# cfdeinza/reinforcement-learning-rendezvous

Hardware: AMD Instinct MI355X
Metric: env steps/sec (higher is better)
Workload: dtype f64

## Files before the change

### reinforcement_learning_rendezvous_amd/csrc/rdv_fused.h

```cpp
#pragma once
#include "rdv_kernels.h"

namespace rdv {

template <typename ST, bool kDiag, bool kGeneral = false, bool kRaw = false>
__global__ __launch_bounds__(kBlock) void step_kernel(void* ws_hot, const float* actions_hot, const DevParams* __restrict__ Pp, int64_t n_hot,
                                                       uint64_t* stats_hot, float* obs_hot, float* reward_hot, const StepArgs A_rest) {
  const StepArgs A = hot_args(A_rest, ws_hot, actions_hot, n_hot, stats_hot, obs_hot, reward_hot);
  using V = typename Vec4<ST>::type;
  __shared__ __attribute__((aligned(16))) float lds[kBlock * RDV_OBS_DIM];
  const DevParams& P = *Pp;
  const int lane = threadIdx.x & (kWave - 1);
  const int wave_in_block = threadIdx.x >> 6;
  const int64_t lblock = A.xcd_per ? (int64_t)(blockIdx.x & 7) * A.xcd_per + (blockIdx.x >> 3) : (int64_t)blockIdx.x;
  const int64_t i = lblock * kBlock + threadIdx.x;
  const int64_t wave_base = i - lane;
  const int64_t n = A.n;
  const bool active = i < n;
  const int64_t rows = (n - wave_base) < kWave ? (n - wave_base) : kWave;
  float* wl = lds + wave_in_block * (kWave * RDV_OBS_DIM);
  V* ws = reinterpret_cast<V*>(A.ws);

  Env e;
  if (active) load_env<ST>(ws, A.cs, i, e);
  uint64_t* slot = A.stats + (uint64_t)(wave_base / kWave) * kStatWords;
  const uint64_t slot_pre = rows > 0 ? stats_preload(slot, lane) : 0ull;
  float a[RDV_ACT_DIM];
  load_actions(A.actions, wave_base, lane, active, a);

  StepResult r;
  const RowSink my_row{wl + lane * RDV_OBS_DIM};
  const bool stepped = advance<ST, kDiag, kGeneral, kRaw>(A, P, i, active, e, a, r, my_row);
  const bool fin = stepped && r.done;
  stats_update(slot, slot_pre, lane, stepped, fin, r.reason, e.flags, e.k, e.ep_ret, e.sum_dv, e.sum_dw);
  store_step_outputs<true>(A, i, active, fin, r, e, my_row.row);
  bool did_reset = false;
  if (fin) {
    if (A.on_done == RDV_ON_DONE_RESET) {
      const double* row = nullptr;
      if (A.tape_depth > 0) row = A.tape + ((int64_t)(e.episode % (uint32_t)A.tape_depth) * n + i) * RDV_STATE_DIM;
      reset_env<ST>(P, e, A.seed, A.env_id_offset + (uint64_t)i, row);
// ... 15 lines not shown
```

### reinforcement_learning_rendezvous_amd/csrc/rdv_general.hip

```cpp
#include "rdv_fused.h"
#include "rdv_slots.h"
#include "rdv_general.h"

namespace rdv {

constexpr int kGenEnvs = 256;
constexpr int kGenBlock = 512;
template <typename ST>
__global__ __launch_bounds__(kGenBlock) void step_kernel_general(void* ws_hot, const float* actions_hot, const DevParams* __restrict__ Pp, int64_t n_hot,
                                                                 uint64_t* stats_hot, float* obs_hot, float* reward_hot, const StepArgs A_rest) {
  const StepArgs A = hot_args(A_rest, ws_hot, actions_hot, n_hot, stats_hot, obs_hot, reward_hot);
  using V = typename Vec4<ST>::type;
  __shared__ __attribute__((aligned(16))) float stage[kGenEnvs * RDV_OBS_DIM];
  __shared__ double handoff[7 * kGenEnvs];
  const DevParams& P = *Pp;
  const int lane = threadIdx.x & (kWave - 1);
  const int wv = threadIdx.x >> 6;
  const bool env_role = wv < kGenEnvs / kWave;
  const int slot = threadIdx.x & (kGenEnvs - 1);
  const int64_t i = (int64_t)blockIdx.x * kGenEnvs + slot;
  const int64_t wave_base = i - lane;
  const int64_t n = A.n;
  const bool active = i < n;
  const int64_t rows = (n - wave_base) < kWave ? (n - wave_base) : kWave;
  V* ws = reinterpret_cast<V*>(A.ws);

  if (env_role) {
    float* wl = stage + wv * (kWave * RDV_OBS_DIM);
    Env e;
    if (active) load_env<ST>(ws, A.cs, i, e);
    uint64_t* slot_stats = A.stats + (uint64_t)(wave_base / kWave) * kStatWords;
    const uint64_t slot_pre = rows > 0 ? stats_preload(slot_stats, lane) : 0ull;
    float a[RDV_ACT_DIM];
    load_actions(A.actions, wave_base, lane, active, a);
    const bool stepping = active && !(e.flags & FLAG_HALTED);
    Derived d;
    StepCtx c;
    StepResult r;
    r.done = 0; r.reason = 0; r.reward = 0.0f; r.reward64 = 0.0;
    if (stepping) step_env_chaser<ST, true, false>(P, e, a, d, c);
    __syncthreads();
    const RowSink my_row{wl + lane * RDV_OBS_DIM};
    if (stepping) {
#pragma unroll
// ... 14 lines not shown
    if (fin) {
      if (A.on_done == RDV_ON_DONE_RESET) {
        reset_env<ST>(P, e, A.seed, A.env_id_offset + (uint64_t)i, tape_row_of(A.tape, A.tape_depth, n, i, e.episode));
        observation_to(P, e, my_row);
      } else if (A.on_done == RDV_ON_DONE_HALT) {
        e.flags |= FLAG_HALTED;
      }
    }
    wave_lds_fence();
    if (A.stream_rows) store_obs_rows<true>(A.obs, wave_base, rows, lane, wl);
    else store_obs_rows<false>(A.obs, wave_base, rows, lane, wl);
    if (stepping) store_env<ST>(ws, A.cs, i, e, true);
  } else {
    double qt[4], wt[3];
    bool stepping = false;
    if (active) {
      const V c4 = ws[4 * A.cs + i], c5 = ws[5 * A.cs + i], c6 = ws[6 * A.cs + i];
      qt[0] = c4.x; qt[1] = c4.y; qt[2] = c4.z; qt[3] = c4.w;
      wt[0] = c6.x; wt[1] = c6.y; wt[2] = c6.z;
      stepping = !(s2u(c5.z) & FLAG_HALTED);
    }
    if (stepping) {
      step_target<true, false>(P, qt, wt);
#pragma unroll
      for (int k = 0; k < 4; ++k) handoff[k * kGenEnvs + slot] = qt[k];
#pragma unroll
      for (int k = 0; k < 3; ++k) handoff[(4 + k) * kGenEnvs + slot] = wt[k];
    }
    __syncthreads();
  }
}

const char* launch_step_general(bool f32, bool diag, bool partner_waves, int64_t n, dim3 fused_grid, hipStream_t s, const DevParams* dev_params, const StepArgs& A) {
#define RDV_LAUNCH_G(GRID, BLOCK, ...) do { hipLaunchKernelGGL((__VA_ARGS__), GRID, BLOCK, 0, s, A.ws, A.actions, dev_params, A.n, A.stats, A.obs, A.reward, A); \
                                             return #__VA_ARGS__; } while (0)
  if (partner_waves && !diag) {
    const dim3 grid((unsigned)((n + kGenEnvs - 1) / kGenEnvs));
    if (f32) RDV_LAUNCH_G(grid, dim3(kGenBlock), step_kernel_general<float>); else RDV_LAUNCH_G(grid, dim3(kGenBlock), step_kernel_general<double>);
  } else {
    const dim3 block(kBlock);
    if (f32) { if (diag) RDV_LAUNCH_G(fused_grid, block, step_kernel<float, true, true>); else RDV_LAUNCH_G(fused_grid, block, step_kernel<float, false, true>); }
    else { if (diag) RDV_LAUNCH_G(fused_grid, block, step_kernel<double, true, true>); else RDV_LAUNCH_G(fused_grid, block, step_kernel<double, false, true>); }
  }
#undef RDV_LAUNCH_G
}

}
```

### reinforcement_learning_rendezvous_amd/csrc/rdv_hip.hip

```cpp
#include "rdv_device.h"
#include "rdv_policy.h"

#include <hip/hip_runtime.h>

#include <cmath>
#include <cstdarg>
#include <cstdio>
#include <cstdlib>
#include <cstring>
#include <new>
#include <vector>

#include "../../include/rdv.h"

#include "rdv_kernels.h"
#include "rdv_fused.h"
#include "rdv_slots.h"
#include "rdv_step.h"
#include "rdv_cold.h"
#include "rdv_rollout.h"
#include "rdv_step_many.h"
#include "rdv_tiles.h"
#include "rdv_general.h"

// ... 658 lines not shown
  StepArgs A;
  base_args(h, A);
  with_storage(h->storage, [&](auto st) { hipLaunchKernelGGL(reset_kernel<decltype(st)>, grid_for(h->n), dim3(kBlock), 0, s, h->dev_params, A, mask, obs_out, fresh); });
  RDV_HIP(hipGetLastError());
  if (fresh) h->prepared_ok = true;
  h->fresh = false;
  return RDV_OK;
}

int rdv_step(rdv_handle h, const float* actions, const RdvStepOut* out, void* stream) {
  RDV_CHECK_HANDLE(h);
  if (!actions || !out || !out->obs || !out->reward || !out->done)
    return fail(RDV_ERR_INVALID_ARGUMENT, "rdv_step: actions, obs, reward and done are required");
  if (h->fresh) return fail(RDV_ERR_INVALID_ARGUMENT, "rdv_step: call rdv_reset first (state is undefined until reset(), as in the reference)");
  RDV_CHECK_FAULT(h);
  if (misaligned(actions, 8) || misaligned(out->obs, 16))
    return fail(RDV_ERR_INVALID_ARGUMENT, "rdv_step: actions must be 8-byte aligned (any row of a [K,N,6] tape is) and obs 16-byte aligned");
  if (out->diag && misaligned(out->diag, 8)) return fail(RDV_ERR_INVALID_ARGUMENT, "rdv_step: diag must be 8-byte aligned");
  DeviceGuard guard(h->device);
  StepArgs A;
  base_args(h, A);
  A.actions = actions;
  A.obs = out->obs; A.reward = out->reward; A.done = out->done; A.terminal_obs = out->terminal_obs;
  A.episode_return = out->episode_return; A.episode_length = out->episode_length; A.done_reason = out->done_reason;
  A.diag = out->diag; A.eval = out->eval;
  if (A.eval && misaligned(A.eval, 8)) return fail(RDV_ERR_INVALID_ARGUMENT, "rdv_step: eval must be 8-byte aligned");
#ifdef RDV_STAMPS
  A.stamps = h->stamps;
#endif
  hipStream_t s = static_cast<hipStream_t>(stream);
  const bool raw = h->raw_state && !h->general;
  h->raw_state = false;
  const bool split = !A.diag && !A.eval && !h->general && !raw && (h->variant == RDV_VARIANT_SPLIT || (h->variant == RDV_VARIANT_AUTO && h->n <= kSplitAutoMaxEnvs));
#define RDV_LAUNCH(GRID, BLOCK, ...) do { hipLaunchKernelGGL((__VA_ARGS__), GRID, BLOCK, 0, s, A.ws, A.actions, h->dev_params, A.n, A.stats, A.obs, A.reward, A); \
                                           h->last_kernel = #__VA_ARGS__; } while (0)
#define RDV_LAUNCH_X(GRID, BLOCK, ...) RDV_LAUNCH(GRID, BLOCK, __VA_ARGS__)
#define RDV_LAUNCH_BY(GRID, BLOCK, FLAG, K) do {                                                                                   \
    if (f32) { if (FLAG) RDV_LAUNCH_X(GRID, BLOCK, K(float, true)); else RDV_LAUNCH_X(GRID, BLOCK, K(float, false)); }             \
    else { if (FLAG) RDV_LAUNCH_X(GRID, BLOCK, K(double, true)); else RDV_LAUNCH_X(GRID, BLOCK, K(double, false)); } } while (0)
#define RDV_K_SPLIT(ST, B) step_kernel_split<ST, B>
#define RDV_K_PARTS(ST, B) step_kernel_parts<ST, B>
#define RDV_K_FUSED(ST, B) step_kernel<ST, B>
#define RDV_K_RAW(ST, B) step_kernel<ST, B, false, true>
  const bool f32 = h->storage == RDV_STORAGE_F32, dg = A.diag != nullptr || A.eval != nullptr;
  if (split) {
    const dim3 grid((unsigned)((h->n + kSplitEnvs - 1) / kSplitEnvs));
    const dim3 block(kSplitBlock);
    const bool all = h->on_done != RDV_ON_DONE_HALT;
    RDV_LAUNCH_BY(grid, block, all, RDV_K_SPLIT);
  } else {
    dim3 grid = grid_for(h->n), block(kBlock);
    { static const int forced = [] { const char* x = getenv("RDV_STREAM_ROWS"); return x ? atoi(x) : -1; }();
      A.stream_rows = forced >= 0 ? (forced ? 1 : 0) : 1; }
    { static const int forced = [] { const char* x = getenv("RDV_STAGGER"); return x ? atoi(x) : -1; }();
      A.stagger = forced >= 0 ? forced : stagger_by_size(h->n); }
    if (h->xcd_order == 1 || (h->xcd_order < 0 && xcd_order_by_size(h->n))) {
      A.xcd_per = (int32_t)((grid.x + 7) / 8);
      grid = dim3((unsigned)A.xcd_per * 8u);
    }
    if (h->general) {
      h->last_kernel = launch_step_general(f32, dg, h->dev.body_general[1] != 0 && h->split_general != 0, h->n, grid, s, h->dev_params, A);
    } else if (raw) {
      RDV_LAUNCH_BY(grid, block, dg, RDV_K_RAW);
    } else if (!dg && h->variant != RDV_VARIANT_FUSED_INLANE) {
      const bool tiles = h->variant == RDV_VARIANT_FUSED_TILES && h->on_done != RDV_ON_DONE_HALT && h->tape_depth == 0;
      if (tiles) {
        unsigned g = h->tiles_grid ? (unsigned)h->tiles_grid : (unsigned)(h->n_cus * kTilesPerCU + 7) / 8u * 8u;
        const unsigned need = A.xcd_per ? (unsigned)A.xcd_per * 8u : grid.x;
        if (g > need) g = need;
        grid = dim3(g);
        h->last_kernel = launch_step_tiles(f32, grid, s, h->dev_params, A);
      } else {
        const bool all = h->on_done != RDV_ON_DONE_HALT;
        RDV_LAUNCH_BY(grid, block, all, RDV_K_PARTS);
      }
    } else {
      RDV_LAUNCH_BY(grid, block, dg, RDV_K_FUSED);
    }
  }
#undef RDV_K_RAW
#undef RDV_K_FUSED
#undef RDV_K_PARTS
#undef RDV_K_SPLIT
#undef RDV_LAUNCH_BY
#undef RDV_LAUNCH_X
#undef RDV_LAUNCH
  RDV_HIP(hipGetLastError());
  if (h->on_done == RDV_ON_DONE_RESET) h->prepared_ok = false;
// ... 200 lines not shown
```

### reinforcement_learning_rendezvous_amd/csrc/rdv_kernels.h

```cpp
#pragma once

#include "rdv_device.h"

#include <hip/hip_runtime.h>
#include <stdint.h>

#include "../../include/rdv.h"

namespace rdv {

#ifndef RDV_PARTS_WAVES
#define RDV_PARTS_WAVES 3
#endif
constexpr int kBlock = 256;
constexpr int kWave = 64;
constexpr int kChunks = 7;
constexpr int kStatWords = 16;
constexpr int64_t kXcdOrderMaxEnvs = 3145728;
static inline bool xcd_order_by_size(int64_t n) { return n <= kXcdOrderMaxEnvs && n % 65536 == 0; }
constexpr int kTilesPerCU = 3;
static inline int stagger_by_size(int64_t n) { return (n < 229376 || n >= 1310720) ? 0 : n < 393216 ? 6 : 8; }
constexpr int64_t kSplitAutoMaxEnvs = 65536;
enum { ST_STEPS = 0, ST_EPISODES, ST_SUCCESS, ST_COLLIDED, ST_REASON0, ST_REASON1, ST_REASON2, ST_REASON3,
       ST_SUM_LEN, ST_SUM_RET, ST_SUM_DV, ST_SUM_DW };

template <typename ST> struct Vec4;
template <> struct Vec4<float> { using type = float4; };
template <> struct Vec4<double> { using type = double4; };

__device__ __forceinline__ float u2s(uint32_t u, float) { return __uint_as_float(u); }
__device__ __forceinline__ double u2s(uint32_t u, double) { return __longlong_as_double((long long)u); }
__device__ __forceinline__ uint32_t s2u(float s) { return __float_as_uint(s); }
__device__ __forceinline__ uint32_t s2u(double s) { return (uint32_t)__double_as_longlong(s); }

template <typename ST>
__device__ __forceinline__ void unpack_env(const typename Vec4<ST>::type* c, Env& e) {
  e.rc[0] = c[0].x; e.rc[1] = c[0].y; e.rc[2] = c[0].z; e.vc[0] = c[0].w;
  e.vc[1] = c[1].x; e.vc[2] = c[1].y; e.wc[0] = c[1].z; e.wc[1] = c[1].w;
// ... 68 lines not shown
#define RDV_STAMP_FLUSH(wave_id)
#endif

struct StepArgs {
  void* ws;
  uint64_t* stats;
  const float* actions;
  float* obs;
  float* reward;
  uint8_t* done;
  float* terminal_obs;
  float* episode_return;
  int32_t* episode_length;
  uint8_t* done_reason;
  double* diag;
  double* eval;
  const double* tape;
  int64_t n;
  int64_t cs;
  uint64_t seed;
  uint64_t env_id_offset;
  int32_t tape_depth;
  int32_t on_done;
  void* prep;
  uint32_t* prep_tag;
  int32_t xcd_per;
  int32_t stream_rows;
  int32_t stagger;
#ifdef RDV_STAMPS
  unsigned long long* stamps;
#endif
};

__device__ __forceinline__ StepArgs hot_args(const StepArgs& rest, void* ws, const float* actions, int64_t n, uint64_t* stats, float* obs,
                                             float* reward) {
  StepArgs A = rest;
  A.ws = ws; A.actions = actions; A.n = n; A.stats = stats; A.obs = obs; A.reward = reward;
  return A;
}
__device__ __forceinline__ StepArgs wave_outputs(const StepArgs& A, int64_t wave_base) {
  StepArgs Aw = A;
  Aw.reward = A.reward + wave_base; Aw.done = A.done + wave_base;
  Aw.done_reason = A.done_reason ? A.done_reason + wave_base : nullptr;
  Aw.terminal_obs = A.terminal_obs ? A.terminal_obs + wave_base * RDV_OBS_DIM : nullptr;
  Aw.episode_return = A.episode_return ? A.episode_return + wave_base : nullptr;
  Aw.episode_length = A.episode_length ? A.episode_length + wave_base : nullptr;
  return Aw;
}
__device__ __forceinline__ void wave_lds_fence() {
  __builtin_amdgcn_fence(__ATOMIC_ACQ_REL, "wavefront");
  __builtin_amdgcn_wave_barrier();
}

__device__ __forceinline__ void load_actions(const float* __restrict__ actions, int64_t wave_base, int lane, bool active, float* a) {
  const float* row = actions + (wave_base + lane) * RDV_ACT_DIM;
#pragma unroll
  for (int k = 0; k < 3; ++k) {
    float2 v = make_float2(0.0f, 0.0f);
    if (active) v = *reinterpret_cast<const float2*>(row + 2 * k);
    a[2 * k] = v.x; a[2 * k + 1] = v.y;
  }
}

template <typename ST>
struct TileInputs {
  typename Vec4<ST>::type c[kChunks];
  float2 a[3];
  uint64_t slot_pre;
};
template <typename ST>
__device__ __forceinline__ void tile_fetch(const StepArgs& A, int64_t wave_base, int lane, TileInputs<ST>& in) {
// ... 94 lines not shown
      iv = lane == ST_REASON0 ? (uint32_t)__popcll(m_r1) : iv;
      iv = lane == ST_REASON1 ? (uint32_t)__popcll(m_r2) : iv;
      iv = lane == ST_REASON2 ? (uint32_t)__popcll(m_r3) : iv;
      iv = lane == ST_REASON3 ? (uint32_t)__popcll(m_r4) : iv;
      iv = lane == ST_SUM_LEN ? (uint32_t)s_len : iv;
      double dv = s_ret;
      dv = lane == ST_SUM_DV ? s_dv : dv;
      dv = lane == ST_SUM_DW ? s_dw : dv;
      const uint64_t as_int = pre + iv;
      const uint64_t as_real = (uint64_t)__double_as_longlong(__longlong_as_double((long long)pre) + dv);
      slot[lane] = lane <= ST_SUM_LEN ? as_int : as_real;
    }
  } else if (lane == 0) {
    slot[ST_STEPS] = pre + __popcll(m_step);
  }
}

template <typename ST, class Sink, class Pre = NoHook>
__device__ __forceinline__ void advance_all(const DevParams& P, Env& e, const float* a, StepResult& r, Sink&& sink, typename Vec4<ST>::type* packed,
                                            Pre&& pre = Pre()) {
  r.done = 0; r.reason = 0; r.reward = 0.0f; r.reward64 = 0.0;
  Derived d;
  step_env<ST, true, false, false>(P, e, a, r, d, sink, NoHook(), pre);
  if (packed) pack_env<ST>(e, packed);
}

typedef float pin_f4 __attribute__((ext_vector_type(4)));
typedef float pin_f2 __attribute__((ext_vector_type(2)));
struct PinnedInputs {
  pin_f4 c[kChunks];
  pin_f4 a4;
  pin_f2 a2;
  pin_f2 sp;
};
__device__ __forceinline__ void pinned_fetch(const StepArgs& A, int64_t wave_base, int lane, PinnedInputs& in) {
  const int64_t wb = wave_base < A.n ? wave_base : ((A.n - 1) & ~(int64_t)(kWave - 1));
  const int64_t rows = A.n - wb;
  const int l = lane < rows ? lane : 0;
  const pin_f4* wsw = reinterpret_cast<const pin_f4*>(A.ws) + wb + l;
#pragma unroll
  for (int c = 0; c < kChunks; ++c) asm volatile("global_load_dwordx4 %0, %1, off" : "=v"(in.c[c]) : "v"(wsw + c * A.cs));
  const float* row = A.actions + (wb + l) * RDV_ACT_DIM;
  asm volatile("global_load_dwordx4 %0, %2, off\n\tglobal_load_dwordx2 %1, %2, off offset:16" : "=&v"(in.a4), "=&v"(in.a2) : "v"(row));
  const uint64_t* sp = A.stats + (uint64_t)(wb / kWave) * kStatWords + (lane & (kStatWords - 1));
  asm volatile("global_load_dwordx2 %0, %1, off" : "=v"(in.sp) : "v"(sp));
}
__device__ __forceinline__ void pinned_wait_state(PinnedInputs& in) {
  asm volatile("s_waitcnt vmcnt(3)" : "+v"(in.c[0]), "+v"(in.c[1]), "+v"(in.c[2]), "+v"(in.c[3]));
  asm volatile("" : "+v"(in.c[4]), "+v"(in.c[5]), "+v"(in.c[6]));
}
__device__ __forceinline__ void pinned_wait_rest(PinnedInputs& in, double& after) { asm volatile("s_waitcnt vmcnt(0)" : "+v"(in.a4), "+v"(in.a2), "+v"(in.sp), "+v"(after)); }
__device__ __forceinline__ void pinned_unpack(const PinnedInputs& in, Env& e) {
  float4 c[kChunks];
#pragma unroll
  for (int j = 0; j < kChunks; ++j) c[j] = make_float4(in.c[j].x, in.c[j].y, in.c[j].z, in.c[j].w);
  unpack_env<float>(c, e);
}

__device__ __forceinline__ void pinned_state(const StepArgs& A, int64_t wave_base, int lane, PinnedInputs& pin, Env& e) {
  pinned_fetch(A, wave_base, lane, pin);
  pinned_wait_state(pin);
  pinned_unpack(pin, e);
}
__device__ __forceinline__ void pinned_rest(PinnedInputs& pin, double& after, float* a, uint64_t& slot_pre) {
  pinned_wait_rest(pin, after);
  a[0] = pin.a4.x; a[1] = pin.a4.y; a[2] = pin.a4.z; a[3] = pin.a4.w; a[4] = pin.a2.x; a[5] = pin.a2.y;
  slot_pre = ((uint64_t)__float_as_uint(pin.sp.y) << 32) | __float_as_uint(pin.sp.x);
}

template <typename ST>
__device__ __forceinline__ void halt_if_done(const StepArgs& A, bool fin, Env& e, typename Vec4<ST>::type* packed) {
  if (fin && A.on_done == RDV_ON_DONE_HALT) { e.flags |= FLAG_HALTED; if (packed) packed[5].z = u2s(e.flags, ST(0)); }
}

template <bool kTerminalObs>
__device__ __forceinline__ void store_step_outputs(const StepArgs& A, int64_t i, bool active, bool fin, const StepResult& r,
                                                   const Env& e, const float* row) {
  if (active) {
    A.reward[i] = r.reward;
    A.done[i] = (uint8_t)r.done;
    if (A.done_reason)
      A.done_reason[i] = (uint8_t)(r.reason | ((fin && (e.flags & FLAG_COLLIDED)) ? 16 : 0) |
                                   ((fin && (e.flags >> SUCCESS_SHIFT) != 0u) ? 32 : 0));
  }
  if (fin) {
    if (kTerminalObs && A.terminal_obs) {
      float* t = A.terminal_obs + i * RDV_OBS_DIM;
#pragma unroll
      for (int j = 0; j < RDV_OBS_DIM; ++j) t[j] = row[j];
    }
    if (A.episode_return) A.episode_return[i] = (float)e.ep_ret;
    if (A.episode_length) A.episode_length[i] = e.k;
  }
}

// ... 35 lines not shown
```

### reinforcement_learning_rendezvous_amd/csrc/rdv_step.h

```cpp
#pragma once
#include "rdv_kernels.h"
#include "rdv_slots.h"

namespace rdv {

template <typename ST>
__global__ __launch_bounds__(kBlock) void prepare_kernel(const DevParams* __restrict__ Pp, const StepArgs A) {
  using V = typename Vec4<ST>::type;
  const int64_t i = (int64_t)blockIdx.x * kBlock + threadIdx.x;
  if (i >= A.n) return;
  const V c5 = reinterpret_cast<const V*>(A.ws)[5 * A.cs + i];
  refill_whole<ST>(A, *Pp, i, s2u(c5.w));
}

template <typename ST, bool kAll>
__global__ __launch_bounds__(kBlock) __attribute__((amdgpu_waves_per_eu(sizeof(ST) == 4 ? RDV_PARTS_WAVES : 3))) void step_kernel_parts(void* ws_hot, const float* actions_hot, const DevParams* __restrict__ Pp, int64_t n_hot,
                                                             uint64_t* stats_hot, float* obs_hot, float* reward_hot, const StepArgs A_rest) {
  const StepArgs A = hot_args(A_rest, ws_hot, actions_hot, n_hot, stats_hot, obs_hot, reward_hot);
  using V = typename Vec4<ST>::type;
  __shared__ __attribute__((aligned(16))) float lds[kBlock * RDV_OBS_DIM];
  __shared__ uint32_t job_kind[kBlock];
  __shared__ uint32_t job_counter[kBlock];
  __shared__ uint16_t lists[kGroupWaves * kBlock];
  static_assert(kBlock == kGroupEnvs, "refill_pass_lds is written for 256-env workgroups");
  const DevParams& P = *Pp;
  const int lane = threadIdx.x & (kWave - 1);
  const int wave_in_block = __builtin_amdgcn_readfirstlane((int)(threadIdx.x >> 6));
  const int64_t lblock = A.xcd_per ? (int64_t)(blockIdx.x & 7) * A.xcd_per + (blockIdx.x >> 3) : (int64_t)blockIdx.x;
  const int64_t block_base = lblock * kBlock;
  const int64_t wave_base = block_base + wave_in_block * kWave;
  const int64_t n = A.n;
  const int64_t rows = (n - wave_base) < kWave ? (n - wave_base) : kWave;
  const bool active = lane < rows;
  float* wl = lds + wave_in_block * (kWave * RDV_OBS_DIM);
  V* ws = reinterpret_cast<V*>(A.ws);
  const bool resets = A.on_done == RDV_ON_DONE_RESET;
  RDV_STAMP_DECL
  RDV_STAMP(0);
  if (A.stagger && blockIdx.x < 1024u) {
    const int slot = (int)(blockIdx.x >> 8);
    for (int k = 0; k < slot * A.stagger; ++k) __builtin_amdgcn_s_sleep(8);
  }

  {
    V* wsw = ws + wave_base;
    const StepArgs Aw = wave_outputs(A, wave_base);
    Env e;
    uint64_t* slot = A.stats + (uint64_t)(wave_base / kWave) * kStatWords;
    uint64_t slot_pre;
    float a[RDV_ACT_DIM];
    constexpr bool kPinned = kAll && sizeof(ST) == 4;
    PinnedInputs pin;
    if constexpr (kPinned) {
      pinned_state(A, wave_base, lane, pin, e);
    } else if constexpr (kAll) {
      TileInputs<ST> in;
      tile_fetch<ST>(A, wave_base, lane, in);
      unpack_env<ST>(in.c, e);
      slot_pre = in.slot_pre;
#pragma unroll
      for (int k = 0; k < 3; ++k) { a[2 * k] = in.a[k].x; a[2 * k + 1] = in.a[k].y; }
    } else {
      if (active) load_env<ST>(wsw, A.cs, lane, e);
      slot_pre = rows > 0 ? stats_preload(slot, lane) : 0ull;
      load_actions(A.actions + wave_base * RDV_ACT_DIM, 0, lane, active, a);
    }
    RDV_STAMP_STATE(e);
    RDV_STAMP(1);
    StepResult r;
    const RowSink my_row{wl + lane * RDV_OBS_DIM};
    constexpr bool kPack = sizeof(ST) == 4;
    V packed[kChunks];
    bool stepped;
    auto actions_ready = [&](double& after) { if constexpr (kPinned) pinned_rest(pin, after, a, slot_pre); };
    if constexpr (kAll) { advance_all<ST>(P, e, a, r, my_row, kPack ? packed : nullptr, actions_ready); stepped = active; }
    else stepped = advance<ST, false, false, false>(A, P, wave_base + lane, active, e, a, r, my_row, NoHook(), kPack ? packed : nullptr);
    RDV_STAMP(2);
    const bool fin = stepped && r.done;
    stats_update(slot, slot_pre, lane, stepped, fin, r.reason, e.flags, e.k, e.ep_ret, e.sum_dv, e.sum_dw);
    store_step_outputs<true>(Aw, lane, active, fin, r, e, my_row.row);
    const bool to_reset = fin && resets;
    halt_if_done<ST>(A, fin, e, kPack ? packed : nullptr);
    if (resets) {
      job_kind[threadIdx.x] = to_reset ? JOB_REFILL : JOB_NONE;
      job_counter[threadIdx.x] = e.episode;
    }
    if (stepped && !to_reset) { if (kPack) store_chunks<ST>(wsw, A.cs, lane, packed, false); else store_env<ST>(wsw, A.cs, lane, e, false); }
  }
  RDV_STAMP(3);
  if (resets) {
    __syncthreads();
    RDV_STAMP(4);
    LiveStore<ST> L;
    L.ws = ws; L.rows = lds; L.cs = A.cs; L.base = block_base;
    refill_pass_lds<ST>(wave_in_block, lane, P, L, job_kind, job_counter, lists + wave_in_block * kBlock, block_base, n, A.seed,
                        A.env_id_offset, A.tape, A.tape_depth);
    RDV_STAMP(5);
    __syncthreads();
  } else {
    wave_lds_fence();
  }
  RDV_STAMP(6);
  if (A.stream_rows) store_obs_rows<true>(A.obs, wave_base, rows, lane, wl);
  else store_obs_rows<false>(A.obs, wave_base, rows, lane, wl);
  RDV_STAMP(7);
  RDV_STAMP_FLUSH((uint64_t)blockIdx.x * (kBlock / kWave) + wave_in_block)
}

constexpr int kSplitEnvs = 256;
constexpr int kSplitBlock = 512;

template <typename ST, bool kAll>
__global__ __launch_bounds__(kSplitBlock) void step_kernel_split(void* ws_hot, const float* actions_hot, const DevParams* __restrict__ Pp, int64_t n_hot,
                                                       uint64_t* stats_hot, float* obs_hot, float* reward_hot, const StepArgs A_rest) {
  const StepArgs A = hot_args(A_rest, ws_hot, actions_hot, n_hot, stats_hot, obs_hot, reward_hot);
  using V = typename Vec4<ST>::type;
  __shared__ __attribute__((aligned(16))) float stage[kSplitEnvs * RDV_OBS_DIM];
  __shared__ unsigned long long fin_mask[kSplitEnvs / kWave];
  const DevParams& P = *Pp;
  const int lane = threadIdx.x & (kWave - 1);
  const int wv = threadIdx.x >> 6;
  const bool step_role = wv < kSplitEnvs / kWave;
  const int slot_in_block = threadIdx.x & (kSplitEnvs - 1);
  const int64_t i = (int64_t)blockIdx.x * kSplitEnvs + slot_in_block;
  const int64_t wave_base = i - lane;
  const int64_t n = A.n;
  const bool active = i < n;
  const int64_t rows = (n - wave_base) < kWave ? (n - wave_base) : kWave;
  V* ws = reinterpret_cast<V*>(A.ws);
  const bool resets = A.on_done == RDV_ON_DONE_RESET;
  RDV_STAMP_DECL
  RDV_STAMP(0);

  if (step_role) {
    __builtin_amdgcn_s_setprio(2);
    float* wl = stage + wv * (kWave * RDV_OBS_DIM);
    Env e;
    StepResult r;
    uint64_t* slot = A.stats + (uint64_t)(wave_base / kWave) * kStatWords;
    uint64_t slot_pre;
    float a[RDV_ACT_DIM];
    constexpr bool kPinned = kAll && sizeof(ST) == 4;
    PinnedInputs pin;
    if constexpr (kPinned) {
      pinned_state(A, wave_base, lane, pin, e);
    } else if constexpr (kAll) {
      TileInputs<ST> in;
      tile_fetch<ST>(A, wave_base, lane, in);
      unpack_env<ST>(in.c, e);
      slot_pre = in.slot_pre;
#pragma unroll
      for (int k = 0; k < 3; ++k) { a[2 * k] = in.a[k].x; a[2 * k + 1] = in.a[k].y; }
    } else {
      if (active) load_env<ST>(ws, A.cs, i, e);
      slot_pre = stats_preload(slot, lane);
      load_actions(A.actions, wave_base, lane, active, a);
    }
    RDV_STAMP_STATE(e);
    RDV_STAMP(1);
    float obs_r[RDV_OBS_DIM];
    float* my_row = wl + lane * RDV_OBS_DIM;
    constexpr bool kPack = sizeof(ST) == 4;
    V packed[kChunks];
    auto row_sink = [&](int j, float v) { obs_r[j] = v; my_row[j] = v; };
    bool stepped;
    auto actions_ready = [&](double& after) { if constexpr (kPinned) pinned_rest(pin, after, a, slot_pre); };
    if constexpr (kAll) { advance_all<ST>(P, e, a, r, row_sink, kPack ? packed : nullptr, actions_ready); stepped = active; }
    else stepped = advance<ST, false>(A, P, i, active, e, a, r, row_sink, NoHook(), kPack ? packed : nullptr);
    RDV_STAMP(2);
    const bool fin = stepped && r.done;
    const bool to_reset = fin && resets;
    const unsigned long long m_reset = __ballot(to_reset);
    if (lane == 0) fin_mask[wv] = m_reset;
    halt_if_done<ST>(A, fin, e, kPack ? packed : nullptr);
    if (stepped && !to_reset) { if (kPack) store_chunks<ST, true>(ws, A.cs, i, packed, false); else store_env<ST>(ws, A.cs, i, e, false); }
    RDV_STAMP(3);
    __syncthreads();
    RDV_STAMP(4);
    stats_update(slot, slot_pre, lane, stepped, fin, r.reason, e.flags, e.k, e.ep_ret, e.sum_dv, e.sum_dw);
    store_step_outputs<true>(A, i, active, fin, r, e, obs_r);
    if (m_reset == 0ull) store_obs_rows<true>(A.obs, wave_base, rows, lane, wl);
    RDV_STAMP(5);
    RDV_STAMP(6);
  } else {
    Env ne;
    if (resets && active) {
      const V c5 = ws[5 * A.cs + i];
      ne.episode = s2u(c5.w);
      RDV_STAMP(1);
      const double* row = nullptr;
      if (A.tape_depth > 0) row = A.tape + ((int64_t)(ne.episode % (uint32_t)A.tape_depth) * n + i) * RDV_STATE_DIM;
      reset_state<ST, false>(P, ne, A.seed, A.env_id_offset + (uint64_t)i, row);
      reset_aux<ST>(P, ne);
      RDV_STAMP(2);
    }
    RDV_STAMP(3);
    __syncthreads();
    RDV_STAMP(4);
    const unsigned long long m_reset = fin_mask[wv - kSplitEnvs / kWave];
    if (m_reset != 0ull) {
      float* wl = stage + (wv - kSplitEnvs / kWave) * (kWave * RDV_OBS_DIM);
      if (active && ((m_reset >> lane) & 1ull)) {
        float robs[RDV_OBS_DIM];
        canon_rest<ST>(ne);
        observation(P, ne, robs);
        store_env<ST, true>(ws, A.cs, i, ne, true);
#pragma unroll
        for (int j = 0; j < RDV_OBS_DIM; ++j) wl[lane * RDV_OBS_DIM + j] = robs[j];
      }
      wave_lds_fence();
      RDV_STAMP(5);
      store_obs_rows<true>(A.obs, wave_base, rows, lane, wl);
    }
    RDV_STAMP(6);
  }
  RDV_STAMP(7);
  RDV_STAMP_FLUSH((uint64_t)blockIdx.x * 8 + wv)
}

}
```

### reinforcement_learning_rendezvous_amd/csrc/rdv_tiles.hip

```cpp
#include "rdv_kernels.h"
#include "rdv_slots.h"
#include "rdv_tiles.h"

namespace rdv {

template <typename ST>
__device__ __forceinline__ void tile_touch(TileInputs<ST>& in) {
#pragma unroll
  for (int c = 0; c < kChunks; ++c) asm volatile("" : "+v"(in.c[c].x), "+v"(in.c[c].y), "+v"(in.c[c].z), "+v"(in.c[c].w));
#pragma unroll
  for (int k = 0; k < 3; ++k) asm volatile("" : "+v"(in.a[k].x), "+v"(in.a[k].y));
  asm volatile("" : "+v"(in.slot_pre));
}

#ifndef RDV_TILES_WAVES
#define RDV_TILES_WAVES 3
#endif
template <typename ST>
__global__ __launch_bounds__(kBlock) __attribute__((amdgpu_waves_per_eu(sizeof(ST) == 4 ? RDV_TILES_WAVES : 2))) void step_kernel_tiles(void* ws_hot, const float* actions_hot, const DevParams* __restrict__ Pp, int64_t n_hot,
                                                             uint64_t* stats_hot, float* obs_hot, float* reward_hot, const StepArgs A_rest) {
  const StepArgs A = hot_args(A_rest, ws_hot, actions_hot, n_hot, stats_hot, obs_hot, reward_hot);
  using V = typename Vec4<ST>::type;
  __shared__ __attribute__((aligned(16))) float lds[kBlock * RDV_OBS_DIM];
  __shared__ uint32_t job_kind[kBlock];
  __shared__ uint32_t job_counter[kBlock];
  __shared__ uint16_t lists[kGroupWaves * kBlock];
  const int lane0 = threadIdx.x & (kWave - 1);
  const int wave_in_block = __builtin_amdgcn_readfirstlane((int)(threadIdx.x >> 6));
  const int64_t n = A.n;
  const int64_t n_tiles = (n + kBlock - 1) / kBlock;
  const int64_t stride = A.xcd_per ? (int64_t)(gridDim.x >> 3) : (int64_t)gridDim.x;
  const int64_t first = A.xcd_per ? (int64_t)(blockIdx.x >> 3) : (int64_t)blockIdx.x;
  const int64_t limit = A.xcd_per ? (int64_t)A.xcd_per : n_tiles;
  const int64_t origin = A.xcd_per ? (int64_t)(blockIdx.x & 7) * A.xcd_per : 0;
  float* wl = lds + wave_in_block * (kWave * RDV_OBS_DIM);
  V* ws = reinterpret_cast<V*>(A.ws);
  const bool resets = A.on_done == RDV_ON_DONE_RESET;

#ifdef RDV_STAMPS
  unsigned long long ph_[12] = {0, 0, 0, 0, 0, 0, 0, 0, 0, 0, 0, 0}, t_prev_ = 0;
  ph_[8] = __builtin_amdgcn_s_memrealtime();
#define TILE_PHASE(k) do { __builtin_amdgcn_sched_barrier(0); const unsigned long long now_ = __builtin_readcyclecounter(); ph_[k] += now_ - t_prev_; t_prev_ = now_; __builtin_amdgcn_sched_barrier(0); } while (0)
  t_prev_ = __builtin_readcyclecounter();
#else
#define TILE_PHASE(k)
#endif
  int64_t lt = first;
  bool have = lt < limit && origin + lt < n_tiles;
  TileInputs<ST> in;
  if (have) tile_fetch<ST>(A, (origin + lt) * kBlock + wave_in_block * kWave, lane0, in);
#pragma clang loop unroll(disable)
  while (have) {
    int lane = lane0;
    asm volatile("" : "+v"(lane));
// ... 50 lines not shown
      if (stepped && !to_reset) store_env<ST>(wsw, A.cs, lane, e, false);
    }
    TILE_PHASE(3);
    if (resets) {
      __syncthreads();
      TILE_PHASE(4);
      LiveStore<ST> L;
      L.ws = ws; L.rows = lds; L.cs = A.cs; L.base = block_base;
      refill_pass_lds<ST>(wave_in_block, lane, P, L, job_kind, job_counter, lists + wave_in_block * kBlock, block_base, n, A.seed,
                          A.env_id_offset, nullptr, 0);
      TILE_PHASE(5);
      __syncthreads();
      TILE_PHASE(6);
    } else {
      wave_lds_fence();
    }
    tile_touch<ST>(in);
    TILE_PHASE(11);
    if (A.stream_rows) store_obs_rows<true>(A.obs, wave_base, rows, lane, wl);
    else store_obs_rows<false>(A.obs, wave_base, rows, lane, wl);
    wave_lds_fence();
    TILE_PHASE(7);
  }
#ifdef RDV_STAMPS
  if (A.stamps && lane0 == 0) {
    ph_[9] = __builtin_amdgcn_s_memrealtime();
    unsigned long long* row = A.stamps + ((uint64_t)blockIdx.x * (kBlock / kWave) + wave_in_block) * 12;
    for (int k = 0; k < 12; ++k) row[k] = ph_[k];
  }
#endif
}

const char* launch_step_tiles(bool f32, dim3 grid, hipStream_t s, const DevParams* dev_params, const StepArgs& A) {
  if (f32) hipLaunchKernelGGL(step_kernel_tiles<float>, grid, dim3(kBlock), 0, s, A.ws, A.actions, dev_params, A.n, A.stats, A.obs, A.reward, A);
  else hipLaunchKernelGGL(step_kernel_tiles<double>, grid, dim3(kBlock), 0, s, A.ws, A.actions, dev_params, A.n, A.stats, A.obs, A.reward, A);
  return f32 ? "step_kernel_tiles<float>" : "step_kernel_tiles<double>";
}

}
```

Baseline: 10.31 billion.

## Pack hot kernel args and defer loading rest of StepArgs from kernarg segment

Changes the kernel signature so the hot prefix carries cs and a packed mode word (tape depth, on_done, stagger, xcd ordering) in place of obs/reward pointers. The remaining StepArgs fields are read from the kernarg segment later via manual scalar loads, after the state loads have been issued, and the kernarg cache lines are warmed with scalar loads. The reset role in the split kernel now uses an asm load of the episode word. The aim is to shorten the kernel prologue's scalar-load latency before state fetches begin, at the cost of fragile kernarg offset assumptions.

```diff
diff --git a/reinforcement_learning_rendezvous_amd/csrc/rdv_fused.h b/reinforcement_learning_rendezvous_amd/csrc/rdv_fused.h
--- a/reinforcement_learning_rendezvous_amd/csrc/rdv_fused.h
+++ b/reinforcement_learning_rendezvous_amd/csrc/rdv_fused.h
@@ -4,9 +4,8 @@
 namespace rdv {
 
 template <typename ST, bool kDiag, bool kGeneral = false, bool kRaw = false>
-__global__ __launch_bounds__(kBlock) void step_kernel(void* ws_hot, const float* actions_hot, const DevParams* __restrict__ Pp, int64_t n_hot,
-                                                       uint64_t* stats_hot, float* obs_hot, float* reward_hot, const StepArgs A_rest) {
-  const StepArgs A = hot_args(A_rest, ws_hot, actions_hot, n_hot, stats_hot, obs_hot, reward_hot);
+__global__ __launch_bounds__(kBlock) void step_kernel(RDV_HOT_PARAMS) {
+  const StepArgs A = hot_args(A_rest, RDV_HOT_HEAD);
   using V = typename Vec4<ST>::type;
   __shared__ __attribute__((aligned(16))) float lds[kBlock * RDV_OBS_DIM];
   const DevParams& P = *Pp;
diff --git a/reinforcement_learning_rendezvous_amd/csrc/rdv_general.hip b/reinforcement_learning_rendezvous_amd/csrc/rdv_general.hip
--- a/reinforcement_learning_rendezvous_amd/csrc/rdv_general.hip
+++ b/reinforcement_learning_rendezvous_amd/csrc/rdv_general.hip
@@ -7,9 +7,8 @@
 constexpr int kGenEnvs = 256;
 constexpr int kGenBlock = 512;
 template <typename ST>
-__global__ __launch_bounds__(kGenBlock) void step_kernel_general(void* ws_hot, const float* actions_hot, const DevParams* __restrict__ Pp, int64_t n_hot,
-                                                                 uint64_t* stats_hot, float* obs_hot, float* reward_hot, const StepArgs A_rest) {
-  const StepArgs A = hot_args(A_rest, ws_hot, actions_hot, n_hot, stats_hot, obs_hot, reward_hot);
+__global__ __launch_bounds__(kGenBlock) void step_kernel_general(RDV_HOT_PARAMS) {
+  const StepArgs A = hot_args(A_rest, RDV_HOT_HEAD);
   using V = typename Vec4<ST>::type;
   __shared__ __attribute__((aligned(16))) float stage[kGenEnvs * RDV_OBS_DIM];
   __shared__ double handoff[7 * kGenEnvs];
@@ -90,7 +89,7 @@
 }
 
 const char* launch_step_general(bool f32, bool diag, bool partner_waves, int64_t n, dim3 fused_grid, hipStream_t s, const DevParams* dev_params, const StepArgs& A) {
-#define RDV_LAUNCH_G(GRID, BLOCK, ...) do { hipLaunchKernelGGL((__VA_ARGS__), GRID, BLOCK, 0, s, A.ws, A.actions, dev_params, A.n, A.stats, A.obs, A.reward, A); \
+#define RDV_LAUNCH_G(GRID, BLOCK, ...) do { hipLaunchKernelGGL((__VA_ARGS__), GRID, BLOCK, 0, s, RDV_HOT_LAUNCH_ARGS(A, dev_params)); \
                                              return #__VA_ARGS__; } while (0)
   if (partner_waves && !diag) {
     const dim3 grid((unsigned)((n + kGenEnvs - 1) / kGenEnvs));
diff --git a/reinforcement_learning_rendezvous_amd/csrc/rdv_hip.hip b/reinforcement_learning_rendezvous_amd/csrc/rdv_hip.hip
--- a/reinforcement_learning_rendezvous_amd/csrc/rdv_hip.hip
+++ b/reinforcement_learning_rendezvous_amd/csrc/rdv_hip.hip
@@ -714,7 +714,7 @@
   const bool raw = h->raw_state && !h->general;
   h->raw_state = false;
   const bool split = !A.diag && !A.eval && !h->general && !raw && (h->variant == RDV_VARIANT_SPLIT || (h->variant == RDV_VARIANT_AUTO && h->n <= kSplitAutoMaxEnvs));
-#define RDV_LAUNCH(GRID, BLOCK, ...) do { hipLaunchKernelGGL((__VA_ARGS__), GRID, BLOCK, 0, s, A.ws, A.actions, h->dev_params, A.n, A.stats, A.obs, A.reward, A); \
+#define RDV_LAUNCH(GRID, BLOCK, ...) do { hipLaunchKernelGGL((__VA_ARGS__), GRID, BLOCK, 0, s, RDV_HOT_LAUNCH_ARGS(A, h->dev_params)); \
                                            h->last_kernel = #__VA_ARGS__; } while (0)
 #define RDV_LAUNCH_X(GRID, BLOCK, ...) RDV_LAUNCH(GRID, BLOCK, __VA_ARGS__)
 #define RDV_LAUNCH_BY(GRID, BLOCK, FLAG, K) do {                                                                                   \
@@ -735,7 +735,7 @@
     { static const int forced = [] { const char* x = getenv("RDV_STREAM_ROWS"); return x ? atoi(x) : -1; }();
       A.stream_rows = forced >= 0 ? (forced ? 1 : 0) : 1; }
     { static const int forced = [] { const char* x = getenv("RDV_STAGGER"); return x ? atoi(x) : -1; }();
-      A.stagger = forced >= 0 ? forced : stagger_by_size(h->n); }
+      A.stagger = forced >= 0 ? (forced < kModeStaggerMax ? forced : kModeStaggerMax) : stagger_by_size(h->n); }
     if (h->xcd_order == 1 || (h->xcd_order < 0 && xcd_order_by_size(h->n))) {
       A.xcd_per = (int32_t)((grid.x + 7) / 8);
       grid = dim3((unsigned)A.xcd_per * 8u);
diff --git a/reinforcement_learning_rendezvous_amd/csrc/rdv_kernels.h b/reinforcement_learning_rendezvous_amd/csrc/rdv_kernels.h
--- a/reinforcement_learning_rendezvous_amd/csrc/rdv_kernels.h
+++ b/reinforcement_learning_rendezvous_amd/csrc/rdv_kernels.h
@@ -3,7 +3,9 @@
 #include "rdv_device.h"
 
 #include <hip/hip_runtime.h>
+#include <stddef.h>
 #include <stdint.h>
+#include <utility>
 
 #include "../../include/rdv.h"
 
@@ -138,11 +140,103 @@
 #endif
 };
 
-__device__ __forceinline__ StepArgs hot_args(const StepArgs& rest, void* ws, const float* actions, int64_t n, uint64_t* stats, float* obs,
-                                             float* reward) {
+#ifndef RDV_HEAD_PRELOAD
+#define RDV_HEAD_PRELOAD 1
+#endif
+#ifndef RDV_HEAD_WARM
+#define RDV_HEAD_WARM 0
+#endif
+constexpr int kModeOnDoneShift = 32, kModeStaggerShift = 34, kModeXcdShift = 42;
+constexpr int kModeStaggerMax = 255;
+inline __host__ __device__ uint64_t hot_mode(const StepArgs& A) {
+  return (uint64_t)(uint32_t)A.tape_depth | (uint64_t)((uint32_t)A.on_done & 3u) << kModeOnDoneShift |
+         (uint64_t)((uint32_t)A.stagger & (uint32_t)kModeStaggerMax) << kModeStaggerShift | (uint64_t)(uint32_t)A.xcd_per << kModeXcdShift;
+}
+#if RDV_HEAD_PRELOAD
+#define RDV_HOT_PARAMS void *ws_hot, const float *actions_hot, const DevParams *__restrict__ Pp, int64_t n_hot, uint64_t *stats_hot, int64_t cs_hot, uint64_t mode_hot, const StepArgs A_rest
+#define RDV_HOT_LAUNCH_ARGS(A, P) (A).ws, (A).actions, (P), (A).n, (A).stats, (A).cs, ::rdv::hot_mode(A), (A)
+#define RDV_HOT_HEAD hot_head(ws_hot, actions_hot, n_hot, stats_hot, cs_hot, mode_hot)
+constexpr int kRestOffset = 7 * 8;
+static_assert(alignof(StepArgs) == 8, "kRestOffset: A_rest follows the hot parameters without padding");
+__device__ __forceinline__ StepArgs hot_head(void* ws, const float* actions, int64_t n, uint64_t* stats, int64_t cs, uint64_t mode) {
+  StepArgs H = {};
+  H.ws = ws; H.actions = actions; H.n = n; H.stats = stats; H.cs = cs;
+  H.tape_depth = (int32_t)(uint32_t)mode; H.on_done = (int32_t)((mode >> kModeOnDoneShift) & 3u);
+  H.stagger = (int32_t)((mode >> kModeStaggerShift) & (uint64_t)kModeStaggerMax); H.xcd_per = (int32_t)(mode >> kModeXcdShift);
+  return H;
+}
+__device__ __forceinline__ StepArgs hot_merge(StepArgs A, const StepArgs& H) {
+  A.ws = H.ws; A.actions = H.actions; A.n = H.n; A.stats = H.stats; A.cs = H.cs;
+  A.tape_depth = H.tape_depth; A.on_done = H.on_done; A.stagger = H.stagger; A.xcd_per = H.xcd_per;
+  return A;
+}
+__device__ __forceinline__ StepArgs hot_args(const StepArgs& rest, const StepArgs& H) { return hot_merge(rest, H); }
+__device__ __forceinline__ StepArgs hot_rest(const StepArgs& rest, const StepArgs& H) {
+  typedef __attribute__((address_space(4))) const uint64_t* kernarg_ptr;
+  static_assert(sizeof(StepArgs) % 8 == 0 && kRestOffset % 8 == 0, "hot_rest copies 8-byte words");
+  kernarg_ptr k = (kernarg_ptr)__builtin_amdgcn_kernarg_segment_ptr();
+  asm volatile("" : "+s"(k));
+  uint64_t w[sizeof(StepArgs) / 8];
+#pragma unroll
+  for (size_t j = 0; j < sizeof(StepArgs) / 8; ++j) w[j] = k[kRestOffset / 8 + j];
+  StepArgs A;
+  __builtin_memcpy(&A, w, sizeof(StepArgs));
+#define RDV_REST_GLOBAL(f) A.f = (decltype(A.f))(void*)(__attribute__((address_space(1))) void*)w[offsetof(StepArgs, f) / 8]
+  RDV_REST_GLOBAL(obs); RDV_REST_GLOBAL(reward); RDV_REST_GLOBAL(done); RDV_REST_GLOBAL(terminal_obs); RDV_REST_GLOBAL(episode_return);
+  RDV_REST_GLOBAL(episode_length); RDV_REST_GLOBAL(done_reason); RDV_REST_GLOBAL(diag); RDV_REST_GLOBAL(eval); RDV_REST_GLOBAL(tape);
+  RDV_REST_GLOBAL(prep); RDV_REST_GLOBAL(prep_tag);
+#ifdef RDV_STAMPS
+  RDV_REST_GLOBAL(stamps);
+#endif
+#undef RDV_REST_GLOBAL
+  return hot_merge(A, H);
+}
+#else
+#define RDV_HOT_PARAMS void *ws_hot, const float *actions_hot, const DevParams *__restrict__ Pp, int64_t n_hot, uint64_t *stats_hot, float *obs_hot, float *reward_hot, const StepArgs A_rest
+#define RDV_HOT_LAUNCH_ARGS(A, P) (A).ws, (A).actions, (P), (A).n, (A).stats, (A).obs, (A).reward, (A)
+#define RDV_HOT_HEAD hot_head(A_rest, ws_hot, actions_hot, n_hot, stats_hot, obs_hot, reward_hot)
+__device__ __forceinline__ StepArgs hot_head(const StepArgs& rest, void* ws, const float* actions, int64_t n, uint64_t* stats, float* obs, float* reward) {
   StepArgs A = rest;
   A.ws = ws; A.actions = actions; A.n = n; A.stats = stats; A.obs = obs; A.reward = reward;
   return A;
+}
+__device__ __forceinline__ StepArgs hot_args(const StepArgs&, const StepArgs& H) { return H; }
+__device__ __forceinline__ StepArgs hot_rest(const StepArgs&, const StepArgs& H) { return H; }
+#endif
+
+__device__ __forceinline__ const DevParams* param_block(const DevParams* Pp) {
+  if constexpr (RDV_HEAD_WARM != 0) {
+    __attribute__((address_space(4))) const DevParams* q = (__attribute__((address_space(4))) const DevParams*)Pp;
+    asm("" : "+s"(q));
+    return (const DevParams*)q;
+  } else {
+    return Pp;
+  }
+}
+template <int kOffset>
+__device__ __forceinline__ void scalar_touch(const void* p, uint32_t& sink) { asm volatile("s_load_dword %0, %1, %2" : "+s"(sink) : "s"(p), "n"(kOffset)); }
+template <int... kLine>
+__device__ __forceinline__ void scalar_warm_lines(const void* p, uint32_t& sink, std::integer_sequence<int, kLine...>) { (scalar_touch<64 * kLine>(p, sink), ...); }
+#if RDV_HEAD_PRELOAD
+constexpr int kRestLines = (kRestOffset + (int)sizeof(StepArgs) + 63) / 64 - 1;
+template <int... kLine>
+__device__ __forceinline__ void scalar_warm_rest(uint32_t& sink, std::integer_sequence<int, kLine...>) {
+  const void* k = (const void*)__builtin_amdgcn_kernarg_segment_ptr();
+  (scalar_touch<64 * (kLine + 1)>(k, sink), ...);
+}
+#endif
+constexpr size_t kWarmBytes = offsetof(DevParams, body_inertia);
+static_assert(kWarmBytes % 4 == 0 && kWarmBytes <= sizeof(DevParams) && sizeof(DevParams) - kWarmBytes == sizeof(double) * 44 + sizeof(int32_t) * 2,
+              "scalar_warm: the general rigid bodies' section is the tail of DevParams and nothing else lies behind body_inertia");
+__device__ __forceinline__ void scalar_warm(const DevParams* p, uint32_t& sink) {
+  sink = 0;
+#if RDV_HEAD_PRELOAD
+  scalar_warm_rest(sink, std::make_integer_sequence<int, kRestLines>());
+#endif
+  if constexpr (RDV_HEAD_WARM != 0) scalar_warm_lines(p, sink, std::make_integer_sequence<int, (int)((kWarmBytes + 63) / 64)>());
+}
+__device__ __forceinline__ void scalar_warm_done(uint32_t sink) {
+  if constexpr (RDV_HEAD_WARM != 0 || RDV_HEAD_PRELOAD != 0) asm volatile("s_waitcnt lgkmcnt(0)" : : "s"(sink));
 }
 __device__ __forceinline__ StepArgs wave_outputs(const StepArgs& A, int64_t wave_base) {
   StepArgs Aw = A;
@@ -303,6 +397,7 @@
   pin_f4 a4;
   pin_f2 a2;
   pin_f2 sp;
+  uint32_t warm;
 };
 __device__ __forceinline__ void pinned_fetch(const StepArgs& A, int64_t wave_base, int lane, PinnedInputs& in) {
   const int64_t wb = wave_base < A.n ? wave_base : ((A.n - 1) & ~(int64_t)(kWave - 1));
@@ -320,7 +415,10 @@
   asm volatile("s_waitcnt vmcnt(3)" : "+v"(in.c[0]), "+v"(in.c[1]), "+v"(in.c[2]), "+v"(in.c[3]));
   asm volatile("" : "+v"(in.c[4]), "+v"(in.c[5]), "+v"(in.c[6]));
 }
-__device__ __forceinline__ void pinned_wait_rest(PinnedInputs& in, double& after) { asm volatile("s_waitcnt vmcnt(0)" : "+v"(in.a4), "+v"(in.a2), "+v"(in.sp), "+v"(after)); }
+__device__ __forceinline__ void pinned_wait_rest(PinnedInputs& in, double& after) {
+  asm volatile("s_waitcnt vmcnt(0)" : "+v"(in.a4), "+v"(in.a2), "+v"(in.sp), "+v"(after));
+  scalar_warm_done(in.warm);
+}
 __device__ __forceinline__ void pinned_unpack(const PinnedInputs& in, Env& e) {
   float4 c[kChunks];
 #pragma unroll
@@ -328,10 +426,15 @@
   unpack_env<float>(c, e);
 }
 
-__device__ __forceinline__ void pinned_state(const StepArgs& A, int64_t wave_base, int lane, PinnedInputs& pin, Env& e) {
-  pinned_fetch(A, wave_base, lane, pin);
+template <bool kRestNow>
+__device__ __forceinline__ StepArgs pinned_state(const StepArgs& H, const StepArgs& rest, const DevParams* Pp, int64_t wave_base, int lane, PinnedInputs& pin, Env& e) {
+  pinned_fetch(H, wave_base, lane, pin);
+  StepArgs A = H;
+  if constexpr (kRestNow) A = hot_rest(rest, H);
+  scalar_warm(Pp, pin.warm);
   pinned_wait_state(pin);
   pinned_unpack(pin, e);
+  return A;
 }
 __device__ __forceinline__ void pinned_rest(PinnedInputs& pin, double& after, float* a, uint64_t& slot_pre) {
   pinned_wait_rest(pin, after);
diff --git a/reinforcement_learning_rendezvous_amd/csrc/rdv_step.h b/reinforcement_learning_rendezvous_amd/csrc/rdv_step.h
--- a/reinforcement_learning_rendezvous_amd/csrc/rdv_step.h
+++ b/reinforcement_learning_rendezvous_amd/csrc/rdv_step.h
@@ -14,56 +14,56 @@
 }
 
 template <typename ST, bool kAll>
-__global__ __launch_bounds__(kBlock) __attribute__((amdgpu_waves_per_eu(sizeof(ST) == 4 ? RDV_PARTS_WAVES : 3))) void step_kernel_parts(void* ws_hot, const float* actions_hot, const DevParams* __restrict__ Pp, int64_t n_hot,
-                                                             uint64_t* stats_hot, float* obs_hot, float* reward_hot, const StepArgs A_rest) {
-  const StepArgs A = hot_args(A_rest, ws_hot, actions_hot, n_hot, stats_hot, obs_hot, reward_hot);
+__global__ __launch_bounds__(kBlock) __attribute__((amdgpu_waves_per_eu(sizeof(ST) == 4 ? RDV_PARTS_WAVES : 3))) void step_kernel_parts(RDV_HOT_PARAMS) {
+  const StepArgs H = RDV_HOT_HEAD;
   using V = typename Vec4<ST>::type;
   __shared__ __attribute__((aligned(16))) float lds[kBlock * RDV_OBS_DIM];
   __shared__ uint32_t job_kind[kBlock];
   __shared__ uint32_t job_counter[kBlock];
   __shared__ uint16_t lists[kGroupWaves * kBlock];
   static_assert(kBlock == kGroupEnvs, "refill_pass_lds is written for 256-env workgroups");
-  const DevParams& P = *Pp;
+  const DevParams* const Pc = param_block(Pp);
+  const DevParams& P = *Pc;
   const int lane = threadIdx.x & (kWave - 1);
   const int wave_in_block = __builtin_amdgcn_readfirstlane((int)(threadIdx.x >> 6));
-  const int64_t lblock = A.xcd_per ? (int64_t)(blockIdx.x & 7) * A.xcd_per + (blockIdx.x >> 3) : (int64_t)blockIdx.x;
+  const int64_t lblock = H.xcd_per ? (int64_t)(blockIdx.x & 7) * H.xcd_per + (blockIdx.x >> 3) : (int64_t)blockIdx.x;
   const int64_t block_base = lblock * kBlock;
   const int64_t wave_base = block_base + wave_in_block * kWave;
-  const int64_t n = A.n;
+  const int64_t n = H.n;
   const int64_t rows = (n - wave_base) < kWave ? (n - wave_base) : kWave;
   const bool active = lane < rows;
   float* wl = lds + wave_in_block * (kWave * RDV_OBS_DIM);
-  V* ws = reinterpret_cast<V*>(A.ws);
-  const bool resets = A.on_done == RDV_ON_DONE_RESET;
+  V* ws = reinterpret_cast<V*>(H.ws);
+  const bool resets = H.on_done == RDV_ON_DONE_RESET;
   RDV_STAMP_DECL
   RDV_STAMP(0);
-  if (A.stagger && blockIdx.x < 1024u) {
+  if (H.stagger && blockIdx.x < 1024u) {
     const int slot = (int)(blockIdx.x >> 8);
-    for (int k = 0; k < slot * A.stagger; ++k) __builtin_amdgcn_s_sleep(8);
-  }
-
+    for (int k = 0; k < slot * H.stagger; ++k) __builtin_amdgcn_s_sleep(8);
+  }
+
+  StepArgs A = H;
   {
     V* wsw = ws + wave_base;
-    const StepArgs Aw = wave_outputs(A, wave_base);
     Env e;
-    uint64_t* slot = A.stats + (uint64_t)(wave_base / kWave) * kStatWords;
+    uint64_t* slot = H.stats + (uint64_t)(wave_base / kWave) * kStatWords;
     uint64_t slot_pre;
     float a[RDV_ACT_DIM];
     constexpr bool kPinned = kAll && sizeof(ST) == 4;
     PinnedInputs pin;
     if constexpr (kPinned) {
-      pinned_state(A, wave_base, lane, pin, e);
+      pinned_state<false>(H, A_rest, Pc, wave_base, lane, pin, e);
     } else if constexpr (kAll) {
       TileInputs<ST> in;
-      tile_fetch<ST>(A, wave_base, lane, in);
+      tile_fetch<ST>(H, wave_base, lane, in);
       unpack_env<ST>(in.c, e);
       slot_pre = in.slot_pre;
 #pragma unroll
       for (int k = 0; k < 3; ++k) { a[2 * k] = in.a[k].x; a[2 * k + 1] = in.a[k].y; }
     } else {
-      if (active) load_env<ST>(wsw, A.cs, lane, e);
+      if (active) load_env<ST>(wsw, H.cs, lane, e);
       slot_pre = rows > 0 ? stats_preload(slot, lane) : 0ull;
-      load_actions(A.actions + wave_base * RDV_ACT_DIM, 0, lane, active, a);
+      load_actions(H.actions + wave_base * RDV_ACT_DIM, 0, lane, active, a);
     }
     RDV_STAMP_STATE(e);
     RDV_STAMP(1);
@@ -78,6 +78,8 @@
     RDV_STAMP(2);
     const bool fin = stepped && r.done;
     stats_update(slot, slot_pre, lane, stepped, fin, r.reason, e.flags, e.k, e.ep_ret, e.sum_dv, e.sum_dw);
+    A = hot_rest(A_rest, H);
+    const StepArgs Aw = wave_outputs(A, wave_base);
     store_step_outputs<true>(Aw, lane, active, fin, r, e, my_row.row);
     const bool to_reset = fin && resets;
     halt_if_done<ST>(A, fin, e, kPack ? packed : nullptr);
@@ -111,24 +113,25 @@
 constexpr int kSplitBlock = 512;
 
 template <typename ST, bool kAll>
-__global__ __launch_bounds__(kSplitBlock) void step_kernel_split(void* ws_hot, const float* actions_hot, const DevParams* __restrict__ Pp, int64_t n_hot,
-                                                       uint64_t* stats_hot, float* obs_hot, float* reward_hot, const StepArgs A_rest) {
-  const StepArgs A = hot_args(A_rest, ws_hot, actions_hot, n_hot, stats_hot, obs_hot, reward_hot);
+__global__ __launch_bounds__(kSplitBlock) void step_kernel_split(RDV_HOT_PARAMS) {
+  const StepArgs H = RDV_HOT_HEAD;
   using V = typename Vec4<ST>::type;
   __shared__ __attribute__((aligned(16))) float stage[kSplitEnvs * RDV_OBS_DIM];
   __shared__ unsigned long long fin_mask[kSplitEnvs / kWave];
-  const DevParams& P = *Pp;
+  const DevParams* const Pc = param_block(Pp);
+  const DevParams& P = *Pc;
   const int lane = threadIdx.x & (kWave - 1);
   const int wv = threadIdx.x >> 6;
   const bool step_role = wv < kSplitEnvs / kWave;
   const int slot_in_block = threadIdx.x & (kSplitEnvs - 1);
   const int64_t i = (int64_t)blockIdx.x * kSplitEnvs + slot_in_block;
   const int64_t wave_base = i - lane;
-  const int64_t n = A.n;
+  const int64_t n = H.n;
   const bool active = i < n;
   const int64_t rows = (n - wave_base) < kWave ? (n - wave_base) : kWave;
-  V* ws = reinterpret_cast<V*>(A.ws);
-  const bool resets = A.on_done == RDV_ON_DONE_RESET;
+  V* ws = reinterpret_cast<V*>(H.ws);
+  const bool resets = H.on_done == RDV_ON_DONE_RESET;
+  StepArgs A = H;
   RDV_STAMP_DECL
   RDV_STAMP(0);
 
@@ -137,24 +140,26 @@
     float* wl = stage + wv * (kWave * RDV_OBS_DIM);
     Env e;
     StepResult r;
-    uint64_t* slot = A.stats + (uint64_t)(wave_base / kWave) * kStatWords;
+    uint64_t* slot = H.stats + (uint64_t)(wave_base / kWave) * kStatWords;
     uint64_t slot_pre;
     float a[RDV_ACT_DIM];
     constexpr bool kPinned = kAll && sizeof(ST) == 4;
     PinnedInputs pin;
     if constexpr (kPinned) {
-      pinned_state(A, wave_base, lane, pin, e);
+      A = pinned_state<true>(H, A_rest, Pc, wave_base, lane, pin, e);
     } else if constexpr (kAll) {
       TileInputs<ST> in;
-      tile_fetch<ST>(A, wave_base, lane, in);
+      tile_fetch<ST>(H, wave_base, lane, in);
+      A = hot_rest(A_rest, H);
       unpack_env<ST>(in.c, e);
       slot_pre = in.slot_pre;
 #pragma unroll
       for (int k = 0; k < 3; ++k) { a[2 * k] = in.a[k].x; a[2 * k + 1] = in.a[k].y; }
     } else {
-      if (active) load_env<ST>(ws, A.cs, i, e);
+      if (active) load_env<ST>(ws, H.cs, i, e);
       slot_pre = stats_preload(slot, lane);
-      load_actions(A.actions, wave_base, lane, active, a);
+      load_actions(H.actions, wave_base, lane, active, a);
+      A = hot_rest(A_rest, H);
     }
     RDV_STAMP_STATE(e);
     RDV_STAMP(1);
@@ -184,9 +189,20 @@
     RDV_STAMP(6);
   } else {
     Env ne;
+    uint32_t episode = 0;
+    if (resets) {
+      uint32_t warm;
+      asm volatile("global_load_dword %0, %1, off offset:%2" : "=v"(episode) : "v"(ws + 5 * H.cs + (active ? i : n - 1)), "n"(3 * sizeof(ST)));
+      A = hot_rest(A_rest, H);
+      scalar_warm(Pc, warm);
+      asm volatile("s_waitcnt vmcnt(0)" : "+v"(episode));
+      scalar_warm_done(warm);
+    }
+#ifdef RDV_STAMPS
+    else A = hot_rest(A_rest, H);
+#endif
     if (resets && active) {
-      const V c5 = ws[5 * A.cs + i];
-      ne.episode = s2u(c5.w);
+      ne.episode = episode;
       RDV_STAMP(1);
       const double* row = nullptr;
       if (A.tape_depth > 0) row = A.tape + ((int64_t)(ne.episode % (uint32_t)A.tape_depth) * n + i) * RDV_STATE_DIM;
diff --git a/reinforcement_learning_rendezvous_amd/csrc/rdv_tiles.hip b/reinforcement_learning_rendezvous_amd/csrc/rdv_tiles.hip
--- a/reinforcement_learning_rendezvous_amd/csrc/rdv_tiles.hip
+++ b/reinforcement_learning_rendezvous_amd/csrc/rdv_tiles.hip
@@ -17,9 +17,8 @@
 #define RDV_TILES_WAVES 3
 #endif
 template <typename ST>
-__global__ __launch_bounds__(kBlock) __attribute__((amdgpu_waves_per_eu(sizeof(ST) == 4 ? RDV_TILES_WAVES : 2))) void step_kernel_tiles(void* ws_hot, const float* actions_hot, const DevParams* __restrict__ Pp, int64_t n_hot,
-                                                             uint64_t* stats_hot, float* obs_hot, float* reward_hot, const StepArgs A_rest) {
-  const StepArgs A = hot_args(A_rest, ws_hot, actions_hot, n_hot, stats_hot, obs_hot, reward_hot);
+__global__ __launch_bounds__(kBlock) __attribute__((amdgpu_waves_per_eu(sizeof(ST) == 4 ? RDV_TILES_WAVES : 2))) void step_kernel_tiles(RDV_HOT_PARAMS) {
+  const StepArgs A = hot_args(A_rest, RDV_HOT_HEAD);
   using V = typename Vec4<ST>::type;
   __shared__ __attribute__((aligned(16))) float lds[kBlock * RDV_OBS_DIM];
   __shared__ uint32_t job_kind[kBlock];
@@ -136,8 +135,8 @@
 }
 
 const char* launch_step_tiles(bool f32, dim3 grid, hipStream_t s, const DevParams* dev_params, const StepArgs& A) {
-  if (f32) hipLaunchKernelGGL(step_kernel_tiles<float>, grid, dim3(kBlock), 0, s, A.ws, A.actions, dev_params, A.n, A.stats, A.obs, A.reward, A);
-  else hipLaunchKernelGGL(step_kernel_tiles<double>, grid, dim3(kBlock), 0, s, A.ws, A.actions, dev_params, A.n, A.stats, A.obs, A.reward, A);
+  if (f32) hipLaunchKernelGGL(step_kernel_tiles<float>, grid, dim3(kBlock), 0, s, RDV_HOT_LAUNCH_ARGS(A, dev_params));
+  else hipLaunchKernelGGL(step_kernel_tiles<double>, grid, dim3(kBlock), 0, s, RDV_HOT_LAUNCH_ARGS(A, dev_params));
   return f32 ? "step_kernel_tiles<float>" : "step_kernel_tiles<double>";
 }
 
```

Result: slower. 10.01 billion (-2.9%).
